# NYXFLOWER/TIP

Measured on AMD Instinct MI355X. Metric: D-D edges aggregated/sec (encoder fwd+bwd), higher is better.
Workload: dtype f32; 1 GPU; TIP-cat full encoder, BioSNAP (645 drugs, 19081 proteins, R=1097), 1xMI355X config; mod=cat, directed_dd_edges=8326508, relations=1097, parallelism=single GPU, launch=hipGraph replay of the captured step, rccl_ranks=0

## Files before the change

tip_amd/csrc/tipk_gemm.hip:

```cpp
#include <stdlib.h>
#include "tipk_common.h"
#include "tipk_slabs.h"

namespace {

typedef float f32x16 __attribute__((ext_vector_type(16)));

constexpr int BK = 32;
constexpr int PAD = 4;

struct GemmArgs {
    int64_t m, n, k, kbatch, ksplit, kchunk;
    const float* a; int64_t a_sm, a_sk, a_sq, a_sz;
    const float* b; int64_t b_sk, b_sn, b_sq, b_sz;
    float* c; int64_t c_sm, c_sz, c_ss;
    const float* c_in; int64_t cin_sm, cin_sz;
    float alpha;
    int relu;
};

typedef unsigned int u32;

__device__ __forceinline__ float ldg(const float* base, u32 byte_off) {
    return *reinterpret_cast<const float*>(reinterpret_cast<const char*>(base) + byte_off);
// ... 214 lines not shown
        const u32 cc = (u32)(col < N ? col : N - 4) * 4u;
        float4 b4[16];
#pragma unroll
        for (int kk = 0; kk < 16; ++kk) b4[kk] = ldg4(b_z, koff[kk] + cc);
        __builtin_amdgcn_sched_barrier(0);
        f32x16 a0 = zero16(), a1 = zero16(), a2 = zero16(), a3 = zero16();
#pragma unroll
        for (int kk = 0; kk < 16; ++kk) {
            a0 = __builtin_amdgcn_mfma_f32_32x32x2f32(av[kk], and_mask(b4[kk].x, kmask(kk)), a0, 0, 0, 0);
            a1 = __builtin_amdgcn_mfma_f32_32x32x2f32(av[kk], and_mask(b4[kk].y, kmask(kk)), a1, 0, 0, 0);
            a2 = __builtin_amdgcn_mfma_f32_32x32x2f32(av[kk], and_mask(b4[kk].z, kmask(kk)), a2, 0, 0, 0);
            a3 = __builtin_amdgcn_mfma_f32_32x32x2f32(av[kk], and_mask(b4[kk].w, kmask(kk)), a3, 0, 0, 0);
        }
        if (col >= N) return;
        float* c_t = c_z + (int64_t)m0 * g.c_sm + nb;
        const float* cin_t = cin_z ? cin_z + (int64_t)m0 * g.cin_sm + nb : nullptr;
        const u32 c_sm = (u32)g.c_sm * 4u, cin_sm = (u32)g.cin_sm * 4u, cb = (u32)row * 16u;
#pragma unroll
        for (int r = 0; r < 16; ++r) {
            const int rl = (r & 3) + 8 * (r >> 2) + 4 * kh;
            if (m0 + rl < M) {
                float4 v = make_float4(g.alpha * a0[r], g.alpha * a1[r], g.alpha * a2[r], g.alpha * a3[r]);
                if (cin_t) {
                    const float4 ci = ldg4(cin_t, (u32)rl * cin_sm + cb);
                    v.x += ci.x; v.y += ci.y; v.z += ci.z; v.w += ci.w;
                }
                if (g.relu) { v.x = fmaxf(v.x, 0.f); v.y = fmaxf(v.y, 0.f); v.z = fmaxf(v.z, 0.f); v.w = fmaxf(v.w, 0.f); }
                *reinterpret_cast<float4*>(reinterpret_cast<char*>(c_t) + ((u32)rl * c_sm + cb)) = v;
            }
        }
        return;
    }
    float bt[THIN_K_NT][16];
#pragma unroll
    for (int j = 0; j < THIN_K_NT; ++j) {
        const int col = nb + 32 * j + row;
        const u32 cc = (u32)(col < N ? col : N - 1) * 4u;
#pragma unroll
        for (int kk = 0; kk < 16; ++kk) bt[j][kk] = ldg(b_z, koff[kk] + cc);
    }
    __builtin_amdgcn_sched_barrier(0);
#pragma unroll
    for (int j = 0; j < THIN_K_NT; ++j) {
        f32x16 acc = zero16();
#pragma unroll
        for (int kk = 0; kk < 16; ++kk)
            acc = __builtin_amdgcn_mfma_f32_32x32x2f32(av[kk], and_mask(bt[j][kk], kmask(kk)), acc, 0, 0, 0);
        store_tile32(g, acc, c_z, cin_z, m0, nb + 32 * j, lane);
    }
}

__device__ __forceinline__ void gemm_thin_m_body(const GemmArgs& g, int64_t block) {
    const int lane = threadIdx.x & 63;
    const int row = lane & 31, kh = lane >> 5;
    const int M = (int)g.m, N = (int)g.n;
    const int n_tiles = (N + 31) / 32;
    const int gw = uniform((int)block * 4 + (int)(threadIdx.x >> 6));
    const int zs = uniform(gw / n_tiles);
    const int nt = gw - zs * n_tiles;
    const int z = uniform(zs / (int)g.ksplit);
    const int slab = zs - z * (int)g.ksplit;
    if (z >= g.kbatch) return;
    const int k_lo = slab * (int)g.kchunk;
    const int k_hi = (k_lo + (int)g.kchunk < (int)g.k) ? k_lo + (int)g.kchunk : (int)g.k;
    const float* __restrict__ a_z = g.a + z * g.a_sz;
    const float* __restrict__ b_z = g.b + z * g.b_sz;
    const int n0 = nt * 32;
    const int col = n0 + row;
    const u32 cc = (u32)(col < N ? col : N - 1) * 4u;
    const u32 a_sk = (u32)g.a_sk * 4u, b_sk = (u32)g.b_sk * 4u;
    const u32 ar = (u32)(row < M ? row : M - 1) * (u32)g.a_sm * 4u;
    float a0[16], b0[16], a1[16], b1[16];
#define TIPK_LOAD_AB(A, B, K0)                                                 \
    _Pragma("unroll") for (int kk = 0; kk < 16; ++kk) {                        \
        const int k_ = (K0) + 2 * kk + kh;                                     \
        const u32 kc_ = (u32)(k_ < k_hi ? k_ : k_hi - 1);                      \
        A[kk] = ldg(a_z, ar + kc_ * a_sk);                                     \
        B[kk] = ldg(b_z, kc_ * b_sk + cc);                                     \
    }                                                                          \
    __builtin_amdgcn_sched_barrier(0);
#define TIPK_MMA(A, B, K0)                                                     \
    _Pragma("unroll") for (int kk = 0; kk < 16; ++kk)                          \
    {                                                                          \
        const u32 mk_ = (K0) + 2 * kk + kh < k_hi ? 0xffffffffu : 0u;          \
        acc = __builtin_amdgcn_mfma_f32_32x32x2f32(and_mask(A[kk], mk_), and_mask(B[kk], mk_), acc, 0, 0, 0); \
    }                                                                          \
    __builtin_amdgcn_sched_barrier(0);
    f32x16 acc = zero16();
    if (k_lo < k_hi) {
        TIPK_LOAD_AB(a0, b0, k_lo)
#pragma unroll 1
        for (int k0 = k_lo; k0 < k_hi; k0 += 64) {
            TIPK_LOAD_AB(a1, b1, k0 + 32)
            TIPK_MMA(a0, b0, k0)
            TIPK_LOAD_AB(a0, b0, k0 + 64)
            TIPK_MMA(a1, b1, k0 + 32)
        }
    }
#undef TIPK_LOAD_AB
#undef TIPK_MMA
    float* c_z = g.c + z * g.c_sz + (int64_t)slab * g.c_ss;
    const float* cin_z = g.c_in ? g.c_in + z * g.cin_sz : nullptr;
    store_tile32(g, acc, c_z, cin_z, 0, n0, lane);
}

__device__ __forceinline__ void gemm_kk_body(const GemmArgs& g, int64_t block) {
    const int lane = threadIdx.x & 63;
    const int row = lane & 31, kh = lane >> 5;
    const int M = (int)g.m, N = (int)g.n;
    const int m_tiles = (M + 31) / 32;
    const int gw = uniform((int)block * 4 + (int)(threadIdx.x >> 6));
    const int zs = uniform(gw / m_tiles);
    const int mt = gw - zs * m_tiles;
    const int z = uniform(zs / (int)g.ksplit);
    const int slab = zs - z * (int)g.ksplit;
    if (z >= g.kbatch) return;
    const int k_lo = slab * (int)g.kchunk;
    const int k_hi = (k_lo + (int)g.kchunk < (int)g.k) ? k_lo + (int)g.kchunk : (int)g.k;
    const int m0 = mt * 32;
    const float* __restrict__ a_z = g.a + z * g.a_sz;
    const float* __restrict__ b_z = g.b + z * g.b_sz;
    const u32 ar = (u32)(m0 + row < M ? m0 + row : M - 1) * (u32)g.a_sm * 4u;
    const u32 br = (u32)(row < N ? row : N - 1) * (u32)g.b_sn * 4u;
    float4 a0[4], b0[4], a1[4], b1[4];
#define TIPK_LOAD_AB(A, B, K0)                                                 \
    _Pragma("unroll") for (int q = 0; q < 4; ++q) {                            \
        const int k_ = (K0) + 8 * q + 4 * kh;                                  \
        const u32 kc_ = (u32)(k_ < k_hi ? k_ : k_hi - 4) * 4u;                 \
        A[q] = ldg4(a_z, ar + kc_);                                            \
        B[q] = ldg4(b_z, br + kc_);                                            \
    }                                                                          \
    __builtin_amdgcn_sched_barrier(0);
#define TIPK_KK_STEP(A, B, K0)                                                 \
    _Pragma("unroll") for (int q = 0; q < 4; ++q) {                            \
        const u32 mk_ = (K0) + 8 * q + 4 * kh < k_hi ? 0xffffffffu : 0u;       \
        acc = __builtin_amdgcn_mfma_f32_32x32x2f32(and_mask(A[q].x, mk_), and_mask(B[q].x, mk_), acc, 0, 0, 0); \
        acc = __builtin_amdgcn_mfma_f32_32x32x2f32(and_mask(A[q].y, mk_), and_mask(B[q].y, mk_), acc, 0, 0, 0); \
        acc = __builtin_amdgcn_mfma_f32_32x32x2f32(and_mask(A[q].z, mk_), and_mask(B[q].z, mk_), acc, 0, 0, 0); \
        acc = __builtin_amdgcn_mfma_f32_32x32x2f32(and_mask(A[q].w, mk_), and_mask(B[q].w, mk_), acc, 0, 0, 0); \
    }                                                                          \
    __builtin_amdgcn_sched_barrier(0);
    f32x16 acc = zero16();
    if (k_lo < k_hi) {
        TIPK_LOAD_AB(a0, b0, k_lo)
#pragma unroll 1
        for (int k0 = k_lo; k0 < k_hi; k0 += 64) {
            TIPK_LOAD_AB(a1, b1, k0 + 32)
            TIPK_KK_STEP(a0, b0, k0)
            TIPK_LOAD_AB(a0, b0, k0 + 64)
            TIPK_KK_STEP(a1, b1, k0 + 32)
        }
    }
#undef TIPK_LOAD_AB
#undef TIPK_KK_STEP
    float* c_z = g.c + z * g.c_sz + (int64_t)slab * g.c_ss;
    const float* cin_z = g.c_in ? g.c_in + z * g.cin_sz : nullptr;
    store_tile32(g, acc, c_z, cin_z, m0, 0, lane);
}

enum { STREAM_NONE = 0, STREAM_THIN_K = 1, STREAM_THIN_M = 2, STREAM_KK = 3, STREAM_THIN_K4 = 4 };

inline bool thin_k_wide_ok(const GemmArgs& g, int64_t batch) {
    static_assert(THIN_K_NT == 4, "the wide body owns four interleaved tiles");
    if ((g.n & 3) || ((g.b_sk | g.c_sm | g.b_sz | g.c_sz) & 3)) return false;
    if (g.c_in && ((g.cin_sm | g.cin_sz) & 3)) return false;
    return ((reinterpret_cast<uintptr_t>(g.b) | reinterpret_cast<uintptr_t>(g.c) | reinterpret_cast<uintptr_t>(g.c_in)) & 15) == 0;
}

inline int stream_kind(const GemmArgs& g, int64_t batch) {
    if (g.kbatch != 1 || g.k < 1) return STREAM_NONE;
    const bool big = g.m * g.n >= (1 << 20) || g.n * g.k >= (1 << 20) || g.m * g.k >= (1 << 20);
    if (!big) return STREAM_NONE;
    const int64_t lim = 0x3fffffffLL;
    if (g.a_sm < 0 || g.a_sk < 0 || g.b_sk < 0 || g.b_sn < 0 || g.m > lim || g.n > lim || g.k > lim) return STREAM_NONE;
    if ((g.m - 1) * g.a_sm + (g.k - 1) * g.a_sk >= lim || (g.k - 1) * g.b_sk + (g.n - 1) * g.b_sn >= lim) return STREAM_NONE;
    if (g.c_sm < 0 || g.cin_sm < 0 || 32 * g.c_sm >= lim || 32 * g.cin_sm >= lim) return STREAM_NONE;
    if (g.k <= 32 && g.ksplit == 1 && g.b_sn == 1 && (g.m >= 256 || (g.m >= 8 && g.n >= (1 << 16))) && g.n >= 1024)
        return (thin_k_wide_ok(g, batch) && !tipk_option(TIPK_OPT_GEMM_THIN_K_NARROW)) ? STREAM_THIN_K4 : STREAM_THIN_K;
    if (g.m <= 32 && g.b_sn == 1 && g.n >= 1024 && g.k >= 256) return STREAM_THIN_M;
    if (tipk_option(TIPK_OPT_GEMM_STREAM_KK) && g.n <= 32 && g.a_sk == 1 && g.b_sk == 1 && g.m >= 256 && g.k >= 1024 && g.k % 4 == 0 && g.a_sm % 4 == 0 &&
        g.b_sn % 4 == 0 && g.a_sz % 4 == 0 && g.b_sz % 4 == 0 && (reinterpret_cast<uintptr_t>(g.a) & 15) == 0 &&
        (reinterpret_cast<uintptr_t>(g.b) & 15) == 0)
        return STREAM_KK;
    return STREAM_NONE;
}

inline int64_t stream_blocks(int kind, const GemmArgs& g, int64_t batch) {
    int64_t waves = 0;
    if (kind == STREAM_THIN_K || kind == STREAM_THIN_K4) waves = batch * tipk_ceil_div(g.m, 32) * tipk_ceil_div(g.n, 32 * THIN_K_NT);
    if (kind == STREAM_THIN_M) waves = batch * g.ksplit * tipk_ceil_div(g.n, 32);
    if (kind == STREAM_KK) waves = batch * g.ksplit * tipk_ceil_div(g.m, 32);
    return tipk_ceil_div(waves, 4);
}

template <int KIND>
__global__ __launch_bounds__(256) void gemm_stream_kernel(GemmArgs g) {
    if (KIND == STREAM_THIN_K) gemm_thin_k_body<false>(g, blockIdx.x);
    if (KIND == STREAM_THIN_K4) gemm_thin_k_body<true>(g, blockIdx.x);
    if (KIND == STREAM_THIN_M) gemm_thin_m_body(g, blockIdx.x);
    if (KIND == STREAM_KK) gemm_kk_body(g, blockIdx.x);
}

constexpr int GROUP_MAX = TIPK_GROUP_MAX;

struct GemmGroupArgs {
    int count;
    int first_block[GROUP_MAX + 1];
    int cfg[GROUP_MAX];
    int gx[GROUP_MAX], gy[GROUP_MAX];
    GemmArgs g[GROUP_MAX];
};

__global__ __launch_bounds__(256) void gemm_f32_group_kernel(GemmGroupArgs ga) {
    __shared__ __attribute__((aligned(16))) float smem[2 * BK * (160 + 2 * PAD)];
    GemmArgs g = ga.g[0];
    int first = 0, gx = ga.gx[0], gy = ga.gy[0], cfg = ga.cfg[0];
#pragma unroll
    for (int q = 1; q < GROUP_MAX; ++q)
        if (q < ga.count && (int)blockIdx.x >= ga.first_block[q]) {
            g = ga.g[q]; first = ga.first_block[q]; gx = ga.gx[q]; gy = ga.gy[q]; cfg = ga.cfg[q];
        }
    const int local = (int)blockIdx.x - first;
    const int64_t bx = local % gx, by = (local / gx) % gy, bz = local / (gx * gy);
    const bool akf = (cfg & 2) != 0, bkf = (cfg & 1) != 0;
    switch (cfg >= 100 ? cfg : cfg >> 2) {
    case 0: gemm_body<4, 1, 2>(g, bx, by, bz, smem, akf, bkf); break;
    case 1: gemm_body<1, 4, 2>(g, bx, by, bz, smem, akf, bkf); break;
    case 2: gemm_body<2, 2, 2>(g, bx, by, bz, smem, akf, bkf); break;
    case 100 + STREAM_THIN_M: gemm_thin_m_body(g, local); break;
    case 100 + STREAM_KK: gemm_kk_body(g, local); break;
    }
}

template <int WM, int WN, int R = 1>
int launch(const GemmArgs& g, const int64_t (&tiles)[3], int route, hipStream_t st) {
    dim3 grid((unsigned)tiles[0], (unsigned)tiles[1], (unsigned)tiles[2]), block(256);
    const bool akf = (route & TIPK_ROUTE_A_KFAST) != 0, bkf = (route & TIPK_ROUTE_B_KFAST) != 0;
    const bool two = (route & TIPK_ROUTE_TWO_BUFFERS) != 0;
#define TIPK_GEMM_GO(A, B)                                                                              \
    do {                                                                                                \
        if (!two) hipLaunchKernelGGL((gemm_f32_kernel<WM, WN, A, B, 1, R>), grid, block, 0, st, g);     \
        else hipLaunchKernelGGL((gemm_f32_kernel<WM, WN, A, B, (R > 1 ? 1 : 2), R>), grid, block, 0, st, g); \
    } while (0)
    if (akf && bkf) TIPK_GEMM_GO(true, true);
    else if (akf) TIPK_GEMM_GO(true, false);
    else if (bkf) TIPK_GEMM_GO(false, true);
    else TIPK_GEMM_GO(false, false);
#undef TIPK_GEMM_GO
    TIPK_RETURN_LAUNCH();
}

template <int LANES>
__global__ __launch_bounds__(64 * LANES) void sum_slabs_kernel(const float* __restrict__ in, int64_t n_slabs,
                                                               int64_t slab_stride, int64_t count, float alpha,
                                                               int accumulate, const float* __restrict__ row_scale,
                                                               int64_t cols, const float* __restrict__ addend,
                                                               int relu, float* __restrict__ out) {
    __shared__ float red[LANES][64];
    const int e = threadIdx.x & 63, j = threadIdx.x >> 6;
    const int64_t i = (int64_t)blockIdx.x * 64 + e;
    float s = 0.f;
    if (i < count) {
        const float* p = in + i;
        int64_t k = j;
        for (; k + 3 * LANES < n_slabs; k += 4 * LANES) {
            const float v0 = p[k * slab_stride], v1 = p[(k + LANES) * slab_stride];
            const float v2 = p[(k + 2 * LANES) * slab_stride], v3 = p[(k + 3 * LANES) * slab_stride];
            s += v0; s += v1; s += v2; s += v3;
        }
        for (; k < n_slabs; k += LANES) s += p[k * slab_stride];
    }
    red[j][e] = s;
    __syncthreads();
    if (j == 0 && i < count) {
        s = red[0][e];
#pragma unroll
        for (int q = 1; q < LANES; ++q) s += red[q][e];
        s *= alpha;
        if (row_scale) s *= row_scale[i / cols];
        if (addend) s += addend[i];
        if (accumulate) s += out[i];
        if (relu) s = fmaxf(s, 0.f);
        out[i] = s;
    }
}

struct SlabGroupArgs {
    int count;
    int first_block[GROUP_MAX + 1];
    SlabArgs s[GROUP_MAX];
};

__global__ __launch_bounds__(1024) void sum_slabs_group_kernel(SlabGroupArgs sa) {
    __shared__ float red[1024];
    SlabArgs a = sa.s[0];
    int first = 0;
#pragma unroll
    for (int q = 1; q < GROUP_MAX; ++q)
        if (q < sa.count && (int)blockIdx.x >= sa.first_block[q]) { a = sa.s[q]; first = sa.first_block[q]; }
    slab_sum_body(a, (int)blockIdx.x - first, red);
}

constexpr int WGK_MAX = 4, WGK_SUMS = 3, WGK_WAVES = 16;

struct WgkJob {
    const float* a; int64_t a_sm, a_sk, a_sq, a_sz;
    const float* b; int64_t b_sk, b_sn, b_sq, b_sz;
    const float* a2; int64_t a2_sm, a2_sk;
    const float* b2; int64_t b2_sk, b2_sn;
    float* c; int64_t c_sm, c_sz;
    const float* c_in; int64_t cin_sm, cin_sz;
    const float* gate; int64_t gate_sm, gate_sz;
    int m, n, k, k2, kbatch;
    int mt, nt;
    int tiles_q, n_kt, per, nw;
    int vec1, vec2;
    float alpha; int relu;
};
struct WgkArgs {
    int n_gemm, n_sum;
    int first[WGK_MAX + WGK_SUMS + 1];
    WgkJob g[WGK_MAX];
    SlabArgs s[WGK_SUMS];
};

__global__ __launch_bounds__(1024) void gemm_wgk_group_kernel(WgkArgs wa) {
    __shared__ __attribute__((aligned(16))) float red[WGK_WAVES * 1024];
    const int blk = (int)blockIdx.x;
    if (blk >= wa.first[WGK_MAX]) {
        SlabArgs sa = wa.s[0];
        int first = wa.first[WGK_MAX];
#pragma unroll
        for (int q = 1; q < WGK_SUMS; ++q)
            if (q < wa.n_sum && blk >= wa.first[WGK_MAX + q]) { sa = wa.s[q]; first = wa.first[WGK_MAX + q]; }
        slab_sum_body(sa, blk - first, red);
        return;
    }
    WgkJob g = wa.g[0];
    int first = 0;
#pragma unroll
    for (int q = 1; q < WGK_MAX; ++q)
        if (q < wa.n_gemm && blk >= wa.first[q]) { g = wa.g[q]; first = wa.first[q]; }
    const int local = blk - first;
    const int nt_i = local % g.nt, mt_i = (local / g.nt) % g.mt, z = local / (g.nt * g.mt);
    const int t = threadIdx.x, lane = t & 63, row = lane & 31, kh = lane >> 5;
    const int w = uniform(t >> 6);
    const int m0 = mt_i * 32, n0 = nt_i * 32;
    const int n_first = g.kbatch * g.tiles_q;
    const u32 am = (u32)(m0 + row < g.m ? m0 + row : g.m - 1), bn = (u32)(n0 + row < g.n ? n0 + row : g.n - 1);
    const u32 m_mask = m0 + row < g.m ? 0xffffffffu : 0u;

    f32x16 acc = zero16();
    float a0[16], b0[16], a1[16], b1[16];
    int left0 = 0, left1 = 0;
    auto load = [&](int tile, float (&av)[16], float (&bv)[16], int& left) {
        const bool second = tile >= n_first;
        const int tq = second ? tile - n_first : tile;
        const int q = second ? 0 : tq / g.tiles_q;
        const int kt = second ? tq : tq - q * g.tiles_q;
        const int kk_total = second ? g.k2 : g.k;
        const int k0 = kt * 32;
        left = kk_total - k0 < 32 ? kk_total - k0 : 32;
        const float* ap = second ? g.a2 : g.a + (int64_t)z * g.a_sz + (int64_t)q * g.a_sq;
        const float* bp = second ? g.b2 : g.b + (int64_t)z * g.b_sz + (int64_t)q * g.b_sq;
        const u32 s_am = (u32)(second ? g.a2_sm : g.a_sm), s_ak = (u32)(second ? g.a2_sk : g.a_sk);
        const u32 s_bk = (u32)(second ? g.b2_sk : g.b_sk), s_bn = (u32)(second ? g.b2_sn : g.b_sn);
        const u32 ao = am * s_am, bo = bn * s_bn;
        if (second ? g.vec2 : g.vec1) {
#pragma unroll
            for (int j = 0; j < 4; ++j) {
                const int kb = 16 * kh + 4 * j;
                const u32 kc = (u32)(k0 + (kb < left ? kb : left - 4));
                const float4 xa = ldg4(ap, (ao + kc) * 4u), xb = ldg4(bp, (bo + kc) * 4u);
                av[4 * j] = xa.x; av[4 * j + 1] = xa.y; av[4 * j + 2] = xa.z; av[4 * j + 3] = xa.w;
                bv[4 * j] = xb.x; bv[4 * j + 1] = xb.y; bv[4 * j + 2] = xb.z; bv[4 * j + 3] = xb.w;
            }
            left = -left;
            return;
        }
#pragma unroll
        for (int kk = 0; kk < 16; ++kk) {
            const int kl = 2 * kk + kh;
            const u32 kc = (u32)(k0 + (kl < left ? kl : left - 1));
            av[kk] = ldg(ap, (ao + kc * s_ak) * 4u);
            bv[kk] = ldg(bp, (kc * s_bk + bo) * 4u);
        }
    };
    auto mma = [&](const float (&av)[16], const float (&bv)[16], int left) {
        const int lim = left < 0 ? -left - 16 * kh : left - kh;
        const int step = left < 0 ? 1 : 2;
#pragma unroll
        for (int kk = 0; kk < 16; ++kk)
            acc = __builtin_amdgcn_mfma_f32_32x32x2f32(and_mask(av[kk], step * kk < lim ? m_mask : 0u),
                                                       and_mask(bv[kk], step * kk < lim ? 0xffffffffu : 0u), acc, 0, 0, 0);
    };
    const int t_lo = w * g.per, t_hi = t_lo + g.per < g.n_kt ? t_lo + g.per : g.n_kt;
    if (t_lo < t_hi) {
        load(t_lo, a0, b0, left0);
#pragma unroll 1
        for (int tile = t_lo; tile < t_hi; tile += 2) {
            if (tile + 1 < t_hi) load(tile + 1, a1, b1, left1);
            __builtin_amdgcn_sched_barrier(0);
            mma(a0, b0, left0);
            __builtin_amdgcn_sched_barrier(0);
            if (tile + 1 < t_hi) {
                if (tile + 2 < t_hi) load(tile + 2, a0, b0, left0);
                __builtin_amdgcn_sched_barrier(0);
                mma(a1, b1, left1);
                __builtin_amdgcn_sched_barrier(0);
            }
        }
#pragma unroll
        for (int r = 0; r < 16; ++r) red[w * 1024 + r * 64 + lane] = acc[r];
    }
    __syncthreads();
    {
        float s = g.nw > 0 ? red[t] : 0.f;
        for (int q = 1; q < g.nw; ++q) s += red[q * 1024 + t];
        const int r = t >> 6, l = t & 63;
        const int rr = m0 + (r & 3) + 8 * (r >> 2) + 4 * (l >> 5), cc = n0 + (l & 31);
        if (rr < g.m && cc < g.n) {
            s *= g.alpha;
            if (g.c_in) s += g.c_in[(int64_t)z * g.cin_sz + (int64_t)rr * g.cin_sm + cc];
            if (g.relu) s = fmaxf(s, 0.f);
            if (g.gate && !(g.gate[(int64_t)z * g.gate_sz + (int64_t)rr * g.gate_sm + cc] > 0.f)) s = 0.f;
            g.c[(int64_t)z * g.c_sz + (int64_t)rr * g.c_sm + cc] = s;
        }
    }
}

}

static int fill_args(const tipk_gemm_desc* d, GemmArgs& g) {
    if (!d || d->m < 0 || d->n < 0 || d->k < 0 || d->batch < 0 || d->kbatch < 1 || d->ksplit < 1) return TIPK_EINVAL;
    if (d->m == 0 || d->n == 0 || d->batch == 0) return 1;
    if (!d->c || (d->k > 0 && (!d->a || !d->b))) return TIPK_EINVAL;
    if (d->ksplit > 1 && (d->c_in || d->relu)) return TIPK_EINVAL;
    if (d->a_sm < 0 || d->a_sk < 0 || d->b_sk < 0 || d->b_sn < 0) return TIPK_EINVAL;
    if (128 * d->a_sm + 32 * d->a_sk >= (1LL << 30) || 128 * d->b_sn + 32 * d->b_sk >= (1LL << 30)) return TIPK_EUNSUPPORTED;
    g.m = d->m; g.n = d->n; g.k = d->k; g.kbatch = d->kbatch; g.ksplit = d->ksplit;
    g.kchunk = tipk_ceil_div(tipk_ceil_div(d->k, d->ksplit), BK) * BK;
    if (g.kchunk == 0) g.kchunk = BK;
    g.a = d->a; g.a_sm = d->a_sm; g.a_sk = d->a_sk; g.a_sq = d->a_sq; g.a_sz = d->a_sz;
    g.b = d->b; g.b_sk = d->b_sk; g.b_sn = d->b_sn; g.b_sq = d->b_sq; g.b_sz = d->b_sz;
    g.c = d->c; g.c_sm = d->c_sm; g.c_sz = d->c_sz; g.c_ss = d->c_ss;
    g.c_in = d->c_in; g.cin_sm = d->cin_sm; g.cin_sz = d->cin_sz;
    g.alpha = d->alpha; g.relu = d->relu;
    return TIPK_OK;
}

static int route_of(const tipk_gemm_desc* d, int grouped, GemmArgs& g, int64_t (&tiles)[3]) {
    tiles[0] = tiles[1] = tiles[2] = 0;
    const int rc = fill_args(d, g);
    if (rc != TIPK_OK) return rc > 0 ? TIPK_ROUTE_NONE : rc;
    const int64_t batch = d->batch;
    int kind = tipk_option(TIPK_OPT_GEMM_NO_STREAM) ? STREAM_NONE : stream_kind(g, batch);
    if (grouped && (kind == STREAM_THIN_K || kind == STREAM_THIN_K4)) kind = STREAM_NONE;
    if (kind != STREAM_NONE) {
        if (stream_blocks(kind, g, batch) > (grouped ? 0x3fffffffLL : 0x7fffffffLL)) return TIPK_EUNSUPPORTED;
        g.kbatch = batch;
        return kind == STREAM_THIN_K ? TIPK_ROUTE_THIN_K : kind == STREAM_THIN_K4 ? TIPK_ROUTE_THIN_K4
             : kind == STREAM_THIN_M ? TIPK_ROUTE_THIN_M : TIPK_ROUTE_KK;
    }
    int body = TIPK_ROUTE_TILED_64X64;
    if (g.n <= 32) body = TIPK_ROUTE_TILED_128X32;
    else if (g.m <= 32) body = TIPK_ROUTE_TILED_32X128;
    else if (!grouped && g.m >= 512 && g.n >= 512 && g.ksplit == 1) body = TIPK_ROUTE_TILED_128X128;
    const int bm = body == TIPK_ROUTE_TILED_128X32 || body == TIPK_ROUTE_TILED_128X128 ? 128 : (body == TIPK_ROUTE_TILED_32X128 ? 32 : 64);
    const int bn = body == TIPK_ROUTE_TILED_32X128 || body == TIPK_ROUTE_TILED_128X128 ? 128 : (body == TIPK_ROUTE_TILED_128X32 ? 32 : 64);
    const int64_t gx = tipk_ceil_div(g.n, bn), gy = tipk_ceil_div(g.m, bm), gz = batch * g.ksplit;
    if (gx > (grouped ? 0x7fffffLL : 0x7fffffffLL) || gy > 65535 || gz > 65535) return TIPK_EUNSUPPORTED;
    if (grouped && gx * gy * gz > 0x3fffffffLL) return TIPK_EUNSUPPORTED;
    tiles[0] = gx; tiles[1] = gy; tiles[2] = gz;
    const bool akf = g.a_sk == 1 || g.a_sm != 1;
    const bool bkf = g.b_sk == 1 && g.b_sn != 1;
    const bool one_tile = g.kbatch == 1 && g.kchunk <= BK;
    const bool two = grouped || (body != TIPK_ROUTE_TILED_128X128 && !one_tile);
    return body | (two ? TIPK_ROUTE_TWO_BUFFERS : 0) | (akf ? TIPK_ROUTE_A_KFAST : 0) | (bkf ? TIPK_ROUTE_B_KFAST : 0);
}

static int stream_kind_of_route(int body) {
    return body == TIPK_ROUTE_THIN_K ? STREAM_THIN_K : body == TIPK_ROUTE_THIN_K4 ? STREAM_THIN_K4
         : body == TIPK_ROUTE_THIN_M ? STREAM_THIN_M : body == TIPK_ROUTE_KK ? STREAM_KK : STREAM_NONE;
}

extern "C" int tipk_gemm_route(const tipk_gemm_desc* d, int grouped) {
    GemmArgs g;
    int64_t tiles[3];
    return route_of(d, grouped != 0, g, tiles);
}

extern "C" int tipk_gemm_f32(const tipk_gemm_desc* d, tipk_stream_t stream) {
    GemmArgs g;
    int64_t tiles[3];
    const int route = route_of(d, 0, g, tiles);
    if (route < 0) return route;
    hipStream_t st = (hipStream_t)stream;
    const int body = route & TIPK_ROUTE_BODY_MASK;
    const int kind = stream_kind_of_route(body);
    if (kind != STREAM_NONE) {
        const int64_t blocks = stream_blocks(kind, g, d->batch);
        if (kind == STREAM_THIN_K)
            hipLaunchKernelGGL(gemm_stream_kernel<STREAM_THIN_K>, dim3((unsigned)blocks), dim3(256), 0, st, g);
        else if (kind == STREAM_THIN_K4)
            hipLaunchKernelGGL(gemm_stream_kernel<STREAM_THIN_K4>, dim3((unsigned)blocks), dim3(256), 0, st, g);
        else if (kind == STREAM_THIN_M)
            hipLaunchKernelGGL(gemm_stream_kernel<STREAM_THIN_M>, dim3((unsigned)blocks), dim3(256), 0, st, g);
        else
            hipLaunchKernelGGL(gemm_stream_kernel<STREAM_KK>, dim3((unsigned)blocks), dim3(256), 0, st, g);
        TIPK_RETURN_LAUNCH();
    }
    switch (body) {
    case TIPK_ROUTE_NONE: return TIPK_OK;
    case TIPK_ROUTE_TILED_128X32: return launch<4, 1>(g, tiles, route, st);
    case TIPK_ROUTE_TILED_32X128: return launch<1, 4>(g, tiles, route, st);
    case TIPK_ROUTE_TILED_128X128: return launch<2, 2, 2>(g, tiles, route, st);
    default: return launch<2, 2>(g, tiles, route, st);
    }
}

extern "C" int tipk_gemm_f32_group(const tipk_gemm_desc* descs, int32_t count, tipk_stream_t stream) {
    if (count < 0 || count > GROUP_MAX || (count > 0 && !descs)) return TIPK_EINVAL;
    GemmGroupArgs ga;
    ga.count = 0;
    int64_t blocks = 0;
    for (int i = 0; i < count; ++i) {
        GemmArgs& g = ga.g[ga.count];
        int64_t tiles[3];
        const int route = route_of(descs + i, 1, g, tiles);
        if (route < 0) return route;
        const int body = route & TIPK_ROUTE_BODY_MASK;
        if (body == TIPK_ROUTE_NONE) continue;
        const int kind = stream_kind_of_route(body);
        int64_t nb;
        if (kind != STREAM_NONE) {
            nb = stream_blocks(kind, g, descs[i].batch);
            ga.cfg[ga.count] = 100 + kind;
            ga.gx[ga.count] = 1;
            ga.gy[ga.count] = 1;
        } else {
            const int shape = body == TIPK_ROUTE_TILED_128X32 ? 0 : (body == TIPK_ROUTE_TILED_32X128 ? 1 : 2);
            ga.cfg[ga.count] = shape * 4 + ((route & TIPK_ROUTE_A_KFAST) ? 2 : 0) + ((route & TIPK_ROUTE_B_KFAST) ? 1 : 0);
            ga.gx[ga.count] = (int)tiles[0];
            ga.gy[ga.count] = (int)tiles[1];
            nb = tiles[0] * tiles[1] * tiles[2];
        }
        ga.first_block[ga.count] = (int)blocks;
        blocks += nb;
        if (blocks > 0x3fffffffLL) return TIPK_EUNSUPPORTED;
        ++ga.count;
    }
    if (ga.count == 0) return TIPK_OK;
    ga.first_block[ga.count] = (int)blocks;
    hipLaunchKernelGGL(gemm_f32_group_kernel, dim3((unsigned)blocks), dim3(256), 0, (hipStream_t)stream, ga);
    TIPK_RETURN_LAUNCH();
}

extern "C" int tipk_sum_slabs_group(const tipk_slab_sum_desc* descs, int32_t count, tipk_stream_t stream) {
    if (count < 0 || count > GROUP_MAX || (count > 0 && !descs)) return TIPK_EINVAL;
    SlabGroupArgs sa;
    sa.count = 0;
    int64_t blocks = 0;
    for (int i = 0; i < count; ++i) {
        int rc;
        const int64_t nb = fill_slab_args(descs[i], sa.s[sa.count], &rc);
        if (rc != TIPK_OK) return rc;
        if (nb == 0) continue;
        sa.first_block[sa.count] = (int)blocks;
        blocks += nb;
        if (blocks > 0x3fffffffLL) return TIPK_EUNSUPPORTED;
        ++sa.count;
    }
    if (sa.count == 0) return TIPK_OK;
    sa.first_block[sa.count] = (int)blocks;
    hipLaunchKernelGGL(sum_slabs_group_kernel, dim3((unsigned)blocks), dim3(1024), 0, (hipStream_t)stream, sa);
    TIPK_RETURN_LAUNCH();
}

static int fill_wgk(const tipk_wg_gemm_desc& d, WgkJob& j) {
    const tipk_gemm_desc& p = d.p;
    if (p.m <= 0 || p.n <= 0 || p.k < 0 || p.batch <= 0 || p.kbatch < 1 || p.ksplit != 1) return TIPK_EINVAL;
    if (!p.c || (p.k > 0 && (!p.a || !p.b)) || p.a_sm < 0 || p.a_sk < 0 || p.b_sk < 0 || p.b_sn < 0) return TIPK_EINVAL;
    const bool second = d.a2 != nullptr;
    if (second && (!d.b2 || d.k2 <= 0 || p.batch != 1 || d.a2_sm < 0 || d.a2_sk < 0 || d.b2_sk < 0 || d.b2_sn < 0)) return TIPK_EINVAL;
    const int64_t lim = 1LL << 30;
    if (p.m > lim || p.n > lim || p.k > lim || p.m * p.a_sm + p.k * p.a_sk >= lim || p.k * p.b_sk + p.n * p.b_sn >= lim) return TIPK_EUNSUPPORTED;
    if (second && (d.k2 > lim || p.m * d.a2_sm + d.k2 * d.a2_sk >= lim || d.k2 * d.b2_sk + p.n * d.b2_sn >= lim)) return TIPK_EUNSUPPORTED;
    const int64_t tiles_q = tipk_ceil_div(p.k, 32);
    const int64_t n_kt = p.kbatch * tiles_q + (second ? tipk_ceil_div(d.k2, 32) : 0);
    const int64_t mt = tipk_ceil_div(p.m, 32), nt = tipk_ceil_div(p.n, 32);
    if (n_kt < 1 || n_kt > WGK_WAVES * 4 || mt * nt * p.batch > 4096) return TIPK_EUNSUPPORTED;
    j.a = p.a; j.a_sm = p.a_sm; j.a_sk = p.a_sk; j.a_sq = p.a_sq; j.a_sz = p.a_sz;
    j.b = p.b; j.b_sk = p.b_sk; j.b_sn = p.b_sn; j.b_sq = p.b_sq; j.b_sz = p.b_sz;
    j.a2 = d.a2; j.a2_sm = d.a2_sm; j.a2_sk = d.a2_sk; j.b2 = d.b2; j.b2_sk = d.b2_sk; j.b2_sn = d.b2_sn;
    j.c = p.c; j.c_sm = p.c_sm; j.c_sz = p.c_sz;
    j.c_in = p.c_in; j.cin_sm = p.cin_sm; j.cin_sz = p.cin_sz;
    j.gate = d.gate; j.gate_sm = d.gate_sm; j.gate_sz = d.gate_sz;
    j.m = (int)p.m; j.n = (int)p.n; j.k = (int)p.k; j.k2 = second ? (int)d.k2 : 0; j.kbatch = (int)p.kbatch;
    j.mt = (int)mt; j.nt = (int)nt;
    j.tiles_q = (int)tiles_q; j.n_kt = (int)n_kt;
    j.per = (int)tipk_ceil_div(n_kt, WGK_WAVES);
    j.nw = (int)tipk_ceil_div(n_kt, j.per);
    j.alpha = p.alpha; j.relu = p.relu;
    const auto al16 = [](const void* q) { return (reinterpret_cast<uintptr_t>(q) & 15) == 0; };
    j.vec1 = p.a_sk == 1 && p.b_sk == 1 && p.k % 4 == 0 && ((p.a_sm | p.b_sn | p.a_sq | p.b_sq | p.a_sz | p.b_sz) & 3) == 0 && al16(p.a) && al16(p.b);
    j.vec2 = second && d.a2_sk == 1 && d.b2_sk == 1 && d.k2 % 4 == 0 && ((d.a2_sm | d.b2_sn) & 3) == 0 && al16(d.a2) && al16(d.b2);
    return TIPK_OK;
}

extern "C" int tipk_gemm_wg_group_supported(const tipk_wg_gemm_desc* d) {
    WgkJob j;
    return d && fill_wgk(*d, j) == TIPK_OK;
}

extern "C" int tipk_gemm_wg_group(const tipk_wg_gemm_desc* descs, int32_t count, const tipk_slab_sum_desc* sums,
                                  int32_t n_sums, tipk_stream_t stream) {
    if (count < 0 || count > WGK_MAX || n_sums < 0 || n_sums > WGK_SUMS || (count > 0 && !descs) || (n_sums > 0 && !sums)) return TIPK_EINVAL;
    WgkArgs wa;
    wa.n_gemm = count; wa.n_sum = 0;
    int64_t blocks = 0;
    for (int i = 0; i < count; ++i) {
        const int rc = fill_wgk(descs[i], wa.g[i]);
        if (rc != TIPK_OK) return rc;
        wa.first[i] = (int)blocks;
        blocks += (int64_t)wa.g[i].mt * wa.g[i].nt * descs[i].p.batch;
    }
    for (int i = count; i <= WGK_MAX; ++i) wa.first[i] = (int)blocks;
    for (int i = 0; i < n_sums; ++i) {
        int rc;
        const int64_t nb = fill_slab_args(sums[i], wa.s[wa.n_sum], &rc);
        if (rc != TIPK_OK) return rc;
        if (nb == 0) continue;
        wa.first[WGK_MAX + wa.n_sum] = (int)blocks;
        blocks += nb;
        if (blocks > 0x3fffffffLL) return TIPK_EUNSUPPORTED;
        ++wa.n_sum;
    }
    for (int i = wa.n_sum; i <= WGK_SUMS; ++i) wa.first[WGK_MAX + i] = (int)blocks;
    if (blocks == 0) return TIPK_OK;
    hipLaunchKernelGGL(gemm_wgk_group_kernel, dim3((unsigned)blocks), dim3(1024), 0, (hipStream_t)stream, wa);
    TIPK_RETURN_LAUNCH();
}

extern "C" int tipk_sum_slabs_ex(const float* in, int64_t n_slabs, int64_t slab_stride, int64_t count, float alpha,
                                 int accumulate, const float* row_scale, int64_t cols, const float* addend, int relu,
                                 float* out, tipk_stream_t stream) {
    if (n_slabs < 0 || count < 0 || (row_scale && cols <= 0)) return TIPK_EINVAL;
    if (count == 0) return TIPK_OK;
    if (!out || (n_slabs > 0 && !in)) return TIPK_EINVAL;
    const int64_t blocks = tipk_ceil_div(count, 64);
    if (blocks > 0x7fffffffLL) return TIPK_EUNSUPPORTED;
    if (n_slabs >= 32 && blocks < 2048)
        hipLaunchKernelGGL(sum_slabs_kernel<16>, dim3((unsigned)blocks), dim3(1024), 0, (hipStream_t)stream, in, n_slabs,
                           slab_stride, count, alpha, accumulate, row_scale, cols, addend, relu, out);
    else
        hipLaunchKernelGGL(sum_slabs_kernel<4>, dim3((unsigned)blocks), dim3(256), 0, (hipStream_t)stream, in, n_slabs,
                           slab_stride, count, alpha, accumulate, row_scale, cols, addend, relu, out);
    TIPK_RETURN_LAUNCH();
}

extern "C" int tipk_sum_slabs(const float* in, int64_t n_slabs, int64_t slab_stride, int64_t count, float alpha,
                              int accumulate, float* out, tipk_stream_t stream) {
    return tipk_sum_slabs_ex(in, n_slabs, slab_stride, count, alpha, accumulate, nullptr, 0, nullptr, 0, out, stream);
}
```

Before: 40.21 billion edges/s.

## Add 16x16 quarter-tile MFMA path and K-packing to split-K workgroup GEMM

Refactors the workgroup split-K GEMM body into a template that can use 16x16x4 MFMA tiles when the job has few output tiles, producing four times as many blocks for small GEMMs. It adds a packed mode that processes two kbatch slices with k<=16 per 32-wide K tile, halving wasted padded lanes, and prefetches c_in/gate before the reduction. Separate vec flags are merged into one template specialization, and debug switches are added. The aim is better occupancy and less wasted MFMA work on tiny relation GEMMs, at the cost of more code paths and possible lower per-block efficiency.

```diff
diff --git a/tip_amd/csrc/tipk_gemm.hip b/tip_amd/csrc/tipk_gemm.hip
--- a/tip_amd/csrc/tipk_gemm.hip
+++ b/tip_amd/csrc/tipk_gemm.hip
@@ -540,6 +540,7 @@
 }
 
 constexpr int WGK_MAX = 4, WGK_SUMS = 3, WGK_WAVES = 16;
+constexpr int WGK_QUARTER_MAX = 128;
 
 struct WgkJob {
     const float* a; int64_t a_sm, a_sk, a_sq, a_sz;
@@ -551,16 +552,155 @@
     const float* gate; int64_t gate_sm, gate_sz;
     int m, n, k, k2, kbatch;
     int mt, nt;
-    int tiles_q, n_kt, per, nw;
-    int vec1, vec2;
+    int tiles_q, n_first, n_kt, per, nw;
+    int vec;
+    int quarter, pack;
     float alpha; int relu;
 };
 struct WgkArgs {
     int n_gemm, n_sum;
+    int dbg;
     int first[WGK_MAX + WGK_SUMS + 1];
     WgkJob g[WGK_MAX];
     SlabArgs s[WGK_SUMS];
 };
+
+template <bool QT, bool VEC>
+__device__ __forceinline__ void wgk_body(const WgkJob& g, int local, float* red, int dbg) {
+    constexpr int T = QT ? 16 : 32, L = QT ? 8 : 16, G = 32 / L, NACC = QT ? 4 : 16, NB = QT ? 4 : 2;
+    typedef float acc_t __attribute__((ext_vector_type(NACC)));
+    const int nt_i = local % g.nt, mt_i = (local / g.nt) % g.mt, z = local / (g.nt * g.mt);
+    const int t = threadIdx.x, lane = t & 63, row = lane & (T - 1), kg = lane / T;
+    const int w = uniform(t >> 6);
+    const int m0 = mt_i * T, n0 = nt_i * T;
+    const u32 am = (u32)(m0 + row < g.m ? m0 + row : g.m - 1), bn = (u32)(n0 + row < g.n ? n0 + row : g.n - 1);
+    const u32 m_mask = m0 + row < g.m ? 0xffffffffu : 0u;
+
+    const int er = t >> 6, el = t & 63;
+    const int rr = QT ? m0 + 4 * (el >> 4) + er : m0 + (er & 3) + 8 * (er >> 2) + 4 * (el >> 5), cc = n0 + (el & (T - 1));
+    const bool mine = t < 64 * NACC && rr < g.m && cc < g.n;
+    float cin_v = 0.f, gate_v = 1.f;
+    if (mine && !TIPK_DBG(dbg & 16384)) {
+        if (g.c_in) cin_v = g.c_in[(int64_t)z * g.cin_sz + (int64_t)rr * g.cin_sm + cc];
+        if (g.gate) gate_v = g.gate[(int64_t)z * g.gate_sz + (int64_t)rr * g.gate_sm + cc];
+    }
+
+    acc_t acc;
+#pragma unroll
+    for (int r = 0; r < NACC; ++r) acc[r] = 0.f;
+    const float* const a_1 = g.a + (int64_t)z * g.a_sz, * const b_1 = g.b + (int64_t)z * g.b_sz, * const a_2 = g.a2, * const b_2 = g.b2;
+    const int64_t a_sq = g.a_sq, b_sq = g.b_sq;
+    const u32 am_1 = (u32)g.a_sm, ak_1 = (u32)g.a_sk, bk_1 = (u32)g.b_sk, bn_1 = (u32)g.b_sn;
+    const u32 am_2 = (u32)g.a2_sm, ak_2 = (u32)g.a2_sk, bk_2 = (u32)g.b2_sk, bn_2 = (u32)g.b2_sn;
+    const int k_1 = g.k, k_2 = g.k2, n_first = g.n_first, tiles_q = g.tiles_q, kbatch = g.kbatch, pack = g.pack;
+    auto load = [=](int tile, float (&av)[L], float (&bv)[L], int& lim) __attribute__((always_inline)) {
+        if (TIPK_DBG(dbg & 8192)) {
+#pragma unroll
+            for (int kk = 0; kk < L; ++kk) av[kk] = bv[kk] = (float)(lane + kk);
+            lim = L;
+            return;
+        }
+        const bool second = tile >= n_first;
+        const bool packed = !second && pack;
+        const int tq = second ? tile - n_first : tile;
+        const int q = second ? 0 : packed ? 2 * tq : tq / tiles_q;
+        const int k0 = (second ? tq : packed ? 0 : tq - q * tiles_q) * 32;
+        u32 pick = (u32)uniform(second ? -1 : 0);
+        asm volatile("" : "+s"(pick));
+        const auto sel = [pick](u32 x1, u32 x2) { return (x2 & pick) | (x1 & ~pick); };
+        const auto selp = [pick](const float* p1, const float* p2) {
+            const uint64_t m = ((uint64_t)pick << 32) | pick;
+            typedef const __attribute__((address_space(1))) float* global_ptr;
+            return (const float*)reinterpret_cast<global_ptr>((reinterpret_cast<uint64_t>(p2) & m) | (reinterpret_cast<uint64_t>(p1) & ~m));
+        };
+        const int kk_total = (int)sel((u32)k_1, (u32)k_2);
+        const float* ap = selp(a_1 + (int64_t)q * a_sq, a_2);
+        const float* bp = selp(b_1 + (int64_t)q * b_sq, b_2);
+        const u32 s_am = sel(am_1, am_2), s_ak = sel(ak_1, ak_2), s_bk = sel(bk_1, bk_2), s_bn = sel(bn_1, bn_2);
+        u32 ao = am * s_am, bo = bn * s_bn;
+        if constexpr (VEC) {
+            int kofs = k0 + L * kg;
+            lim = kk_total - kofs;
+            if (packed) {
+                const int up = (L * kg) >> 4;
+                const bool there = q + up < kbatch;
+                kofs &= 15;
+                lim = there ? kk_total - kofs : 0;
+                if (up && there) { ao += (u32)a_sq; bo += (u32)b_sq; }
+            }
+#pragma unroll
+            for (int j = 0; j < L / 4; ++j) {
+                const int kb = kofs + 4 * j;
+                const u32 kc = (u32)(kb < kk_total ? kb : kk_total - 4);
+                const float4 xa = ldg4(ap, (ao + kc) * 4u), xb = ldg4(bp, (bo + kc) * 4u);
+                av[4 * j] = xa.x; av[4 * j + 1] = xa.y; av[4 * j + 2] = xa.z; av[4 * j + 3] = xa.w;
+                bv[4 * j] = xb.x; bv[4 * j + 1] = xb.y; bv[4 * j + 2] = xb.z; bv[4 * j + 3] = xb.w;
+            }
+            return;
+        }
+        const int left = kk_total - k0;
+        lim = (left - kg + G - 1) / G;
+#pragma unroll
+        for (int kk = 0; kk < L; ++kk) {
+            const int kl = G * kk + kg;
+            const u32 kc = (u32)(k0 + (kl < left ? kl : left - 1));
+            av[kk] = ldg(ap, (ao + kc * s_ak) * 4u);
+            bv[kk] = ldg(bp, (kc * s_bk + bo) * 4u);
+        }
+    };
+    auto mma = [&](const float (&av)[L], const float (&bv)[L], int lim) __attribute__((always_inline)) {
+#pragma unroll
+        for (int kk = 0; kk < L; ++kk) {
+            if (TIPK_DBG(dbg & 4096)) {
+                asm volatile("" : : "v"(av[kk]), "v"(bv[kk]));
+                continue;
+            }
+            const float x = and_mask(av[kk], kk < lim ? m_mask : 0u), y = and_mask(bv[kk], kk < lim ? 0xffffffffu : 0u);
+            if constexpr (QT) acc = __builtin_amdgcn_mfma_f32_16x16x4f32(x, y, acc, 0, 0, 0);
+            else acc = __builtin_amdgcn_mfma_f32_32x32x2f32(x, y, acc, 0, 0, 0);
+        }
+    };
+    const int t_lo = w * g.per, t_hi = t_lo + g.per < g.n_kt ? t_lo + g.per : g.n_kt;
+    if (t_lo < t_hi) {
+        float av[NB][L], bv[NB][L];
+        int lim[NB] = {};
+        if constexpr (QT) {
+#pragma unroll
+            for (int i = 0; i < NB; ++i)
+                if (t_lo + i < t_hi) load(t_lo + i, av[i], bv[i], lim[i]);
+            __builtin_amdgcn_sched_barrier(0);
+#pragma unroll
+            for (int i = 0; i < NB; ++i)
+                if (t_lo + i < t_hi) mma(av[i], bv[i], lim[i]);
+        } else {
+            load(t_lo, av[0], bv[0], lim[0]);
+#pragma unroll 1
+            for (int tile = t_lo; tile < t_hi; tile += 2) {
+                if (tile + 1 < t_hi) load(tile + 1, av[1], bv[1], lim[1]);
+                __builtin_amdgcn_sched_barrier(0);
+                mma(av[0], bv[0], lim[0]);
+                __builtin_amdgcn_sched_barrier(0);
+                if (tile + 1 < t_hi) {
+                    if (tile + 2 < t_hi) load(tile + 2, av[0], bv[0], lim[0]);
+                    __builtin_amdgcn_sched_barrier(0);
+                    mma(av[1], bv[1], lim[1]);
+                    __builtin_amdgcn_sched_barrier(0);
+                }
+            }
+        }
+#pragma unroll
+        for (int r = 0; r < NACC; ++r) red[w * (64 * NACC) + r * 64 + lane] = acc[r];
+    }
+    __syncthreads();
+    if (!mine) return;
+    float s = g.nw > 0 ? red[t] : 0.f;
+    for (int q = 1; q < g.nw; ++q) s += red[q * (64 * NACC) + t];
+    s *= g.alpha;
+    if (g.c_in) s += cin_v;
+    if (g.relu) s = fmaxf(s, 0.f);
+    if (g.gate && !(gate_v > 0.f)) s = 0.f;
+    g.c[(int64_t)z * g.c_sz + (int64_t)rr * g.c_sm + cc] = s;
+}
 
 __global__ __launch_bounds__(1024) void gemm_wgk_group_kernel(WgkArgs wa) {
     __shared__ __attribute__((aligned(16))) float red[WGK_WAVES * 1024];
@@ -579,91 +719,12 @@
 #pragma unroll
     for (int q = 1; q < WGK_MAX; ++q)
         if (q < wa.n_gemm && blk >= wa.first[q]) { g = wa.g[q]; first = wa.first[q]; }
-    const int local = blk - first;
-    const int nt_i = local % g.nt, mt_i = (local / g.nt) % g.mt, z = local / (g.nt * g.mt);
-    const int t = threadIdx.x, lane = t & 63, row = lane & 31, kh = lane >> 5;
-    const int w = uniform(t >> 6);
-    const int m0 = mt_i * 32, n0 = nt_i * 32;
-    const int n_first = g.kbatch * g.tiles_q;
-    const u32 am = (u32)(m0 + row < g.m ? m0 + row : g.m - 1), bn = (u32)(n0 + row < g.n ? n0 + row : g.n - 1);
-    const u32 m_mask = m0 + row < g.m ? 0xffffffffu : 0u;
-
-    f32x16 acc = zero16();
-    float a0[16], b0[16], a1[16], b1[16];
-    int left0 = 0, left1 = 0;
-    auto load = [&](int tile, float (&av)[16], float (&bv)[16], int& left) {
-        const bool second = tile >= n_first;
-        const int tq = second ? tile - n_first : tile;
-        const int q = second ? 0 : tq / g.tiles_q;
-        const int kt = second ? tq : tq - q * g.tiles_q;
-        const int kk_total = second ? g.k2 : g.k;
-        const int k0 = kt * 32;
-        left = kk_total - k0 < 32 ? kk_total - k0 : 32;
-        const float* ap = second ? g.a2 : g.a + (int64_t)z * g.a_sz + (int64_t)q * g.a_sq;
-        const float* bp = second ? g.b2 : g.b + (int64_t)z * g.b_sz + (int64_t)q * g.b_sq;
-        const u32 s_am = (u32)(second ? g.a2_sm : g.a_sm), s_ak = (u32)(second ? g.a2_sk : g.a_sk);
-        const u32 s_bk = (u32)(second ? g.b2_sk : g.b_sk), s_bn = (u32)(second ? g.b2_sn : g.b_sn);
-        const u32 ao = am * s_am, bo = bn * s_bn;
-        if (second ? g.vec2 : g.vec1) {
-#pragma unroll
-            for (int j = 0; j < 4; ++j) {
-                const int kb = 16 * kh + 4 * j;
-                const u32 kc = (u32)(k0 + (kb < left ? kb : left - 4));
-                const float4 xa = ldg4(ap, (ao + kc) * 4u), xb = ldg4(bp, (bo + kc) * 4u);
-                av[4 * j] = xa.x; av[4 * j + 1] = xa.y; av[4 * j + 2] = xa.z; av[4 * j + 3] = xa.w;
-                bv[4 * j] = xb.x; bv[4 * j + 1] = xb.y; bv[4 * j + 2] = xb.z; bv[4 * j + 3] = xb.w;
-            }
-            left = -left;
-            return;
-        }
-#pragma unroll
-        for (int kk = 0; kk < 16; ++kk) {
-            const int kl = 2 * kk + kh;
-            const u32 kc = (u32)(k0 + (kl < left ? kl : left - 1));
-            av[kk] = ldg(ap, (ao + kc * s_ak) * 4u);
-            bv[kk] = ldg(bp, (kc * s_bk + bo) * 4u);
-        }
-    };
-    auto mma = [&](const float (&av)[16], const float (&bv)[16], int left) {
-        const int lim = left < 0 ? -left - 16 * kh : left - kh;
-        const int step = left < 0 ? 1 : 2;
-#pragma unroll
-        for (int kk = 0; kk < 16; ++kk)
-            acc = __builtin_amdgcn_mfma_f32_32x32x2f32(and_mask(av[kk], step * kk < lim ? m_mask : 0u),
-                                                       and_mask(bv[kk], step * kk < lim ? 0xffffffffu : 0u), acc, 0, 0, 0);
-    };
-    const int t_lo = w * g.per, t_hi = t_lo + g.per < g.n_kt ? t_lo + g.per : g.n_kt;
-    if (t_lo < t_hi) {
-        load(t_lo, a0, b0, left0);
-#pragma unroll 1
-        for (int tile = t_lo; tile < t_hi; tile += 2) {
-            if (tile + 1 < t_hi) load(tile + 1, a1, b1, left1);
-            __builtin_amdgcn_sched_barrier(0);
-            mma(a0, b0, left0);
-            __builtin_amdgcn_sched_barrier(0);
-            if (tile + 1 < t_hi) {
-                if (tile + 2 < t_hi) load(tile + 2, a0, b0, left0);
-                __builtin_amdgcn_sched_barrier(0);
-                mma(a1, b1, left1);
-                __builtin_amdgcn_sched_barrier(0);
-            }
-        }
-#pragma unroll
-        for (int r = 0; r < 16; ++r) red[w * 1024 + r * 64 + lane] = acc[r];
-    }
-    __syncthreads();
-    {
-        float s = g.nw > 0 ? red[t] : 0.f;
-        for (int q = 1; q < g.nw; ++q) s += red[q * 1024 + t];
-        const int r = t >> 6, l = t & 63;
-        const int rr = m0 + (r & 3) + 8 * (r >> 2) + 4 * (l >> 5), cc = n0 + (l & 31);
-        if (rr < g.m && cc < g.n) {
-            s *= g.alpha;
-            if (g.c_in) s += g.c_in[(int64_t)z * g.cin_sz + (int64_t)rr * g.cin_sm + cc];
-            if (g.relu) s = fmaxf(s, 0.f);
-            if (g.gate && !(g.gate[(int64_t)z * g.gate_sz + (int64_t)rr * g.gate_sm + cc] > 0.f)) s = 0.f;
-            g.c[(int64_t)z * g.c_sz + (int64_t)rr * g.c_sm + cc] = s;
-        }
+    if (g.quarter) {
+        if (g.vec) wgk_body<true, true>(g, blk - first, red, wa.dbg);
+        else wgk_body<true, false>(g, blk - first, red, wa.dbg);
+    } else {
+        if (g.vec) wgk_body<false, true>(g, blk - first, red, wa.dbg);
+        else wgk_body<false, false>(g, blk - first, red, wa.dbg);
     }
 }
 
@@ -835,14 +896,22 @@
     j.c_in = p.c_in; j.cin_sm = p.cin_sm; j.cin_sz = p.cin_sz;
     j.gate = d.gate; j.gate_sm = d.gate_sm; j.gate_sz = d.gate_sz;
     j.m = (int)p.m; j.n = (int)p.n; j.k = (int)p.k; j.k2 = second ? (int)d.k2 : 0; j.kbatch = (int)p.kbatch;
-    j.mt = (int)mt; j.nt = (int)nt;
-    j.tiles_q = (int)tiles_q; j.n_kt = (int)n_kt;
-    j.per = (int)tipk_ceil_div(n_kt, WGK_WAVES);
-    j.nw = (int)tipk_ceil_div(n_kt, j.per);
     j.alpha = p.alpha; j.relu = p.relu;
     const auto al16 = [](const void* q) { return (reinterpret_cast<uintptr_t>(q) & 15) == 0; };
-    j.vec1 = p.a_sk == 1 && p.b_sk == 1 && p.k % 4 == 0 && ((p.a_sm | p.b_sn | p.a_sq | p.b_sq | p.a_sz | p.b_sz) & 3) == 0 && al16(p.a) && al16(p.b);
-    j.vec2 = second && d.a2_sk == 1 && d.b2_sk == 1 && d.k2 % 4 == 0 && ((d.a2_sm | d.b2_sn) & 3) == 0 && al16(d.a2) && al16(d.b2);
+    const bool vec1 = p.a_sk == 1 && p.b_sk == 1 && p.k % 4 == 0 && ((p.a_sm | p.b_sn | p.a_sq | p.b_sq | p.a_sz | p.b_sz) & 3) == 0 && al16(p.a) && al16(p.b);
+    const bool vec2 = second && d.a2_sk == 1 && d.b2_sk == 1 && d.k2 % 4 == 0 && ((d.a2_sm | d.b2_sn) & 3) == 0 && al16(d.a2) && al16(d.b2);
+    const bool legacy = TIPK_DBG(tipk_option(TIPK_OPT_DP_DEBUG) & 32768) != 0;
+    j.quarter = !legacy && 4 * mt * nt * p.batch <= WGK_QUARTER_MAX;
+    j.vec = (vec1 || p.k == 0) && (vec2 || !second);
+    j.pack = !legacy && j.vec && p.k > 0 && p.k <= 16 && p.kbatch > 1 && p.a_sq >= 0 && p.b_sq >= 0 &&
+             p.a_sq + p.m * p.a_sm + p.k < lim && p.b_sq + p.n * p.b_sn + p.k < lim;
+    const int64_t n_first = j.pack ? tipk_ceil_div(p.kbatch, 2) : p.kbatch * tiles_q;
+    const int64_t n_run = n_first + (n_kt - p.kbatch * tiles_q);
+    const int edge = j.quarter ? 16 : 32;
+    j.mt = (int)tipk_ceil_div(p.m, edge); j.nt = (int)tipk_ceil_div(p.n, edge);
+    j.tiles_q = (int)tiles_q; j.n_first = (int)n_first; j.n_kt = (int)n_run;
+    j.per = (int)tipk_ceil_div(n_run, WGK_WAVES);
+    j.nw = (int)tipk_ceil_div(n_run, j.per);
     return TIPK_OK;
 }
 
@@ -856,6 +925,7 @@
     if (count < 0 || count > WGK_MAX || n_sums < 0 || n_sums > WGK_SUMS || (count > 0 && !descs) || (n_sums > 0 && !sums)) return TIPK_EINVAL;
     WgkArgs wa;
     wa.n_gemm = count; wa.n_sum = 0;
+    wa.dbg = TIPK_DBG(tipk_option(TIPK_OPT_DP_DEBUG));
     int64_t blocks = 0;
     for (int i = 0; i < count; ++i) {
         const int rc = fill_wgk(descs[i], wa.g[i]);
```

After: 41.31 billion edges/s, median of 6. 1.03x the previous value.
